# k2kobayashi/crank

Measured on AMD Instinct MI355X. Metric: train frames/sec, higher is better.
Workload: dtype bf16; 1 GPU; vqvae trainer step (all sub-updates), VCC2020-shaped synthetic 80-dim mlfb, 64 utterances x 500 frames per GPU, 14 speakers; trainer=vqvae, global_batch=64, batch_len=500, parallelism=dp1

## Files before the change

crank_amd/_lib.py:

```python
import ctypes
import os
from .config import cfg
from ctypes import c_char_p, c_double, c_float, c_int, c_longlong, c_ulonglong, c_void_p

_HERE = os.path.dirname(os.path.abspath(__file__))
LIB_PATH = cfg.lib_path or os.path.join(_HERE, "libcrank_hip.so")
_lib = None

ERRORS = {1: "invalid argument", 2: "HIP runtime error", 3: "unsupported shape/configuration"}


class NetDesc(ctypes.Structure):
    _fields_ = [
        ("kind", c_int), ("in_ch", c_int), ("out_ch", c_int), ("kernel_size", c_int), ("layers", c_int),
        ("stacks", c_int), ("res_ch", c_int), ("gate_ch", c_int), ("skip_ch", c_int), ("aux_ch", c_int),
        ("conv_ch", c_int), ("causal", c_int), ("use_bias", c_int), ("slope", c_float), ("dropout", c_float),
    ]


COLLATE_MAX_STREAMS = 8


class CollateStream(ctypes.Structure):
    _fields_ = [("src", c_void_p), ("ld", c_int), ("col0", c_int), ("ncols", c_int), ("dst", c_void_p)]


class CollateDesc(ctypes.Structure):
    _fields_ = [
        ("n_streams", c_int), ("streams", CollateStream * COLLATE_MAX_STREAMS), ("utt_start", c_void_p),
        ("utt_spk", c_void_p), ("n_utt", c_int), ("n_spk", c_int), ("lcf0_raw", c_void_p),
        ("spk_lcf0_mean", c_void_p), ("spk_lcf0_std", c_void_p), ("raw", c_void_p), ("raw_start", c_void_p),
        ("fftl", c_int), ("hop", c_int),
    ]


ADAM_MAX_BLOCKS = 4


class AdamBlock(ctypes.Structure):
    _fields_ = [("params", c_void_p), ("grads", c_void_p), ("exp_avg", c_void_p), ("exp_avg_sq", c_void_p),
                ("n", c_longlong), ("lr_dev", c_void_p), ("step_dev", c_void_p)]


class StreamDesc(ctypes.Structure):
    _fields_ = [
        ("n_stacks", c_int), ("in_ch", c_int), ("out_ch", c_int), ("emb_dim", c_int * 3), ("emb_size", c_int * 3),
        ("cb_off", c_longlong * 3), ("enc_base", c_longlong * 3), ("dec_base", c_longlong * 3), ("causal", c_int),
        ("enc_f0", c_int), ("dec_f0", c_int), ("spk_dim", c_int), ("spk_onehot", c_int), ("n_spk", c_int),
        ("spk_off", c_longlong),
    ]


class F0StreamRound(ctypes.Structure):
    _fields_ = [("ids", c_void_p), ("utt", c_void_p), ("range", c_void_p), ("chan_bf", c_void_p), ("chan", c_void_p),
                ("n_ready", c_int), ("total_samples", c_longlong), ("total_channels", c_longlong),
                ("total_frames", c_longlong), ("total_events", c_longlong)]


P, I, LL, ULL, F, D = c_void_p, c_int, c_longlong, c_ulonglong, c_float, c_double

SIGNATURES = {
    "crk_net_create": (P, [ctypes.POINTER(NetDesc)]),
    "crk_net_destroy": (None, [P]),
    "crk_net_param_count": (LL, [P]),
    "crk_net_conv_count": (I, [P]),
    "crk_net_conv_info": (I, [P, I, ctypes.POINTER(c_longlong)]),
    "crk_net_saved_bytes": (LL, [P, I, I]),
    "crk_net_reserve": (I, [P, I, I]),
    "crk_net_scratch_bytes": (LL, [P, I, I]),
    "crk_debug_alloc_count": (LL, []),
    "crk_debug_net_paths": (I, [P, I, I]),
    "crk_debug_net_partials": (LL, [P, I, I, P, LL, P]),
    "crk_seed_next": (I, [P, P, P]),
    "crk_nets_wnorm_bwd": (I, [I, P, P]),
    "crk_nets_prepare": (I, [I, P, P, ULL, P, P]),
    "crk_nets_prepare_models": (I, [I, P, P, P, I, P, P]),
    "crk_net_forward": (I, [P, P, ULL, P, I, P, I, P, I, P, I, I, I, ULL, P]),
    "crk_net_backward": (I, [P, P, ULL, P, P, I, P, I, P, I, P, I, F, P, I, P, I, I, I, ULL, P]),
    "crk_net_backward_scaled": (I, [P, P, ULL, P, P, I, P, I, P, I, P, I, F, P, I, P, I, I, I, ULL, P, P, P]),
    "crk_net_embed_grad_supported": (I, [P, I, I, I]),
    "crk_net_backward_embed": (I, [P, P, ULL, P, P, I, P, I, P, I, P, I, F, P, I, I, I, ULL, P, LL, I, I, I, P, P]),
    "crk_vq_forward": (I, [P, I, P, I, I, I, P, P, I, P, I, P]),
    "crk_vq_forward_fused": (I, [P, I, P, I, P, I, P, I, I, I, P, P, I, P, I, P, P, P, P, P]),
    "crk_vq_image_bytes": (LL, [I, I]),
    "crk_vq_image_build_multi": (I, [I, P, P, I, P, P]),
    "crk_vq_ema_scratch_bytes": (LL, [I, I, I]),
    "crk_vq_ema_stats": (I, [P, I, P, I, I, I, P, P, P, P]),
    "crk_vq_ema_apply": (I, [P, P, P, P, P, I, I, D, D, P]),
    "crk_vq_ema_partial": (I, [P, I, P, I, I, I, P, P]),
    "crk_vq_ema_reduce_multi": (I, [I, P, P, P, P, P, P, P]),
    "crk_vq_ema_apply_multi": (I, [I, P, P, P, P, P, P, P, D, D, P]),
    "crk_vq_ema_partial_multi": (I, [I, P, P, P, P, P, P, P, P]),
    "crk_vq_ema_reduce_size_multi": (I, [I, P, P, P, P, P, P, P, D, D, P]),
    "crk_vq_ema_blend_multi": (I, [I, P, P, P, P, P, P, D, P]),
    "crk_vq_ema_blend_image_multi": (I, [I, P, P, P, P, P, P, D, P, P]),
    "crk_stft_loss_multi_fwd": (I, [P, I, P, I, I, I, I, I, P, P, P, P, F, P, P, P]),
    "crk_stft_loss_multi_fwd_grad": (I, [P, I, P, I, I, I, I, I, P, P, P, P, F, P, P, I, P, P]),
    "crk_stft_loss_multi_bwd": (I, [P, I, P, I, I, I, I, I, P, P, P, P, F, P, P, I, P]),
    "crk_loss_scratch_floats": (I, []),
    "crk_masked_loss_fwd": (I, [P, I, P, I, F, P, LL, I, I, P, P, P]),
    "crk_masked_loss_bwd": (I, [P, I, P, I, F, P, LL, I, I, P, P, P, I, P, I, P]),
    "crk_masked_loss_both_fwd": (I, [P, I, P, I, P, LL, I, P, P, P]),
    "crk_weighted_sum": (I, [I, P, P, F, P, P]),
    "crk_weighted_sum_bwd": (I, [I, P, P, P, P]),
    "crk_recon_supported": (I, [I, I, P, P, P]),
    "crk_stft_twiddle_floats": (LL, [I, I]),
    "crk_stft_twiddles": (I, [I, I, P, P, P]),
    "crk_recon_grad_floats": (LL, [I, I, I, I, P, P]),
    "crk_recon_loss_fwd": (I, [P, I, P, I, P, I, I, I, I, P, P, P, P, F, P, P, P, P]),
    "crk_recon_loss_bwd": (I, [P, I, P, I, P, I, I, I, I, P, P, P, P, P, P, P, P, P, I, P]),
    "crk_masked_loss_bwd_acc": (I, [P, I, P, I, F, P, LL, I, I, P, P, P, I, P, I, P, I, P, P]),
    "crk_vq_commit_bwd": (I, [P, I, P, I, P, LL, I, P, P, P, I, P, I, P, I, P, I, P, I, P]),
    "crk_ce_fwd": (I, [P, I, P, LL, I, I, P, P, P, P]),
    "crk_ce_bwd": (I, [P, LL, I, P, P, P, P]),
    "crk_stft_loss_fwd": (I, [P, I, P, I, I, I, I, I, I, I, P, F, F, I, P, P, P]),
    "crk_stft_loss_bwd": (I, [P, I, P, I, I, I, I, I, I, I, P, F, F, P, P, I, P]),
    "crk_adam_step": (I, [P, P, P, P, LL, P, P, F, F, F, I, P]),
    "crk_adam_step_multi": (I, [I, ctypes.POINTER(AdamBlock), F, F, F, I, P]),
    "crk_radam_step": (I, [P, P, P, P, LL, P, P, D, D, D, I, P]),
    "crk_lamb_step": (I, [P, P, P, P, P, P, I, P, I, P, P, P, P, D, D, D, I, P]),
    "crk_lamb_tile": (I, []),
    "crk_concat_embed": (I, [P, I, I, P, I, I, P, I, P, LL, P, I, P]),
    "crk_embed_bwd_scratch_floats": (LL, [LL, I, I]),
    "crk_embed_bwd": (I, [P, I, I, I, P, LL, I, P, P, P]),
    "crk_concat_embed_run": (I, [P, I, I, P, I, I, P, I, P, LL, LL, P, I, P]),
    "crk_embed_bwd_run": (I, [P, I, I, I, P, LL, LL, I, P, P, P]),
    "crk_logmel_fwd": (I, [P, I, I, I, I, I, I, I, P, P, I, F, P, P, P, I, I, P]),
    "crk_logmel_stream_create": (I, [I, I, I, P, P, I, F, P, P, I, I, I, ctypes.POINTER(c_void_p)]),
    "crk_logmel_stream_destroy": (None, [P]),
    "crk_logmel_stream_state_bytes": (LL, [P]),
    "crk_logmel_stream_max_frames": (I, [P]),
    "crk_logmel_stream_reset": (I, [P, P, I, P]),
    "crk_logmel_stream_push": (I, [P, P, I, P, P, I, I, P, I, P, P]),
    "crk_scaler_apply": (I, [P, I, P, I, LL, I, P, P, I, P]),
    "crk_scaler_workspace_bytes": (LL, [I, I]),
    "crk_scaler_moments": (I, [P, I, I, I, LL, P, P, I, P, LL, P]),
    "crk_scaler_merge": (I, [P, LL, I, I, P, P, P, P, I, P, P, P, P]),
    "crk_hist_accumulate": (I, [P, LL, P, P, P, P, I, I, P, D, D, D, I, P, P, P]),
    "crk_collate_batch": (I, [ctypes.POINTER(CollateDesc), P, I, I, P, P, P, P, P, P, P, P, P]),
    "crk_decode_f0": (I, [P, P, I, I, P, P, D, D, I, P, P, P, P, P, P]),
    "crk_mcd_scratch_bytes": (LL, [I, I, I, I, I]),
    "crk_mcd_fastdtw": (I, [P, P, P, P, I, I, I, I, I, P, P, P, LL, P, P, P]),
    "crk_voc_create": (P, [I, I, I, I, P, I, P]),
    "crk_voc_destroy": (None, [P]),
    "crk_voc_workspace_bytes": (LL, [P, I, I]),
    "crk_voc_forward": (I, [P, P, P, I, I, P, P, P, LL, I, P]),
    "crk_voc_upsample": (I, [P, P, P, I, I, P, P, LL, P]),
    "crk_voc_stream_create": (I, [P, I, I, ctypes.POINTER(c_void_p)]),
    "crk_voc_stream_destroy": (None, [P]),
    "crk_voc_stream_state_bytes": (LL, [P]),
    "crk_voc_stream_lookahead": (I, [P]),
    "crk_voc_stream_reset": (I, [P, P, I, P]),
    "crk_voc_stream_push": (I, [P, P, P, P, P, I, I, P, P, I, P]),
    "crk_world_create": (P, [I, I, D, D, I, I, I]),
    "crk_world_destroy": (None, [P]),
    "crk_world_reserve": (I, [P, LL]),
    "crk_world_workspace_bytes": (LL, [P, I, LL, LL]),
# ... 122 lines not shown
```

crank_amd/csrc/loss_kernels.hip:

```cpp
#include <algorithm>
#include <type_traits>

#include "common.h"

#include "../../include/crank_hip.h"

__device__ __forceinline__ float block_sum_256(float v, float* sh) {
#pragma unroll
  for (int o = 32; o > 0; o >>= 1) v += __shfl_xor(v, o, 64);
  const int tid = threadIdx.x;
  __syncthreads();
  if ((tid & 63) == 0) sh[tid >> 6] = v;
  __syncthreads();
  return sh[0] + sh[1] + sh[2] + sh[3];
}

template <int NC>
__device__ __forceinline__ void sum_partials(const float* part, int stride, int n, float (&s)[NC], float* sh) {
#pragma unroll
  for (int j = 0; j < NC; j++) s[j] = 0.f;
  for (int i = threadIdx.x; i < n; i += 256) {
#pragma unroll
    for (int j = 0; j < NC; j++) s[j] += part[stride * i + j];
  }
// ... 952 lines not shown
            v[0] += a.x * g3; v[1 % V] += a.y * g3; v[2 % V] += a.z * g3; v[3 % V] += a.w * g3;
          } else {
            v[0] += gp[0] * g3;
          }
        }
      }
    }
    if (!p.mask || p.mask[n]) {
      float xv[V], yv[V];
      if (V == 4) {
        const float4 a = *reinterpret_cast<const float4*>(p.x + n * p.ldx + d);
        const float4 c = *reinterpret_cast<const float4*>(p.y + n * p.ldy + d);
        xv[0] = a.x; xv[1 % V] = a.y; xv[2 % V] = a.z; xv[3 % V] = a.w;
        yv[0] = c.x; yv[1 % V] = c.y; yv[2 % V] = c.z; yv[3 % V] = c.w;
      } else {
        xv[0] = p.x[n * p.ldx + d]; yv[0] = p.y[n * p.ldy + d];
      }
#pragma unroll
      for (int j = 0; j < V; j++) {
        const float df = xv[j] - yv[j];
        if (p.g1) v[j] += df > 0.f ? g1 : (df < 0.f ? -g1 : 0.f);
        if (p.g2) v[j] += 2.f * df * g2;
      }
    }
    if (V == 4) *reinterpret_cast<float4*>(p.dx + n * p.lddx + d) = make_float4(v[0], v[1 % V], v[2 % V], v[3 % V]);
    else p.dx[n * p.lddx + d] = v[0];
  }
}

extern "C" int crk_recon_loss_bwd(const float* x, int ldx, const float* y, int ldy, const unsigned char* mask, int B, int T,
                                  int D, int nres, const int* n_fft, const int* hop_length, const int* win_length,
                                  const float* out5, const float* grad, const float* g1, const float* g2, const float* g3,
                                  float* dx, int lddx, void* stream) {
  if (!x || !y || !out5 || !dx || B < 1 || T < 1 || D < 1) return CRK_ERR_ARG;
  if (g3 && (!grad || !crk_recon_supported(T, nres, n_fft, hop_length, win_length))) return CRK_ERR_ARG;
  ReconBP p;
  p.x = x; p.y = y; p.mask = mask; p.ldx = ldx; p.ldy = ldy; p.T = T; p.D = D; p.nres = g3 ? nres : 0;
  p.N = (long)B * T; p.stat = out5; p.g1 = g1; p.g2 = g2; p.g3 = g3; p.dx = dx; p.lddx = lddx;
  const float* g = grad;
  for (int r = 0; r < p.nres; r++) {
    ReconBRes& q = p.r[r];
    q.hop = hop_length[r]; q.span = win_length[r] + RC_SPAN_EXTRA; q.nf = 1 + T / q.hop;
    q.lo = n_fft[r] / 2 - (n_fft[r] - win_length[r]) / 2 + 1;
    q.gc = g;
    g += (size_t)B * q.nf * q.span * D;
  }
  const bool v4 = !((((uintptr_t)x) | ((uintptr_t)y) | ((uintptr_t)dx) | ((uintptr_t)grad)) & 15) && !((D | ldx | ldy | lddx) & 3);
  if (v4) hipLaunchKernelGGL(recon_bwd_kernel<4>, dim3(loss_blocks(p.N * (D / 4))), dim3(256), 0, (hipStream_t)stream, p);
  else hipLaunchKernelGGL(recon_bwd_kernel<1>, dim3(loss_blocks(p.N * D)), dim3(256), 0, (hipStream_t)stream, p);
  CRK_CHECK_LAUNCH();
  return CRK_OK;
}

#define WS_MAX 16
struct WsumP { const float* t[WS_MAX]; float w[WS_MAX]; int n; float c; float* out; const float* g; };
__global__ void weighted_sum_kernel(const WsumP p) {
  float s = 0.f;
#pragma unroll
  for (int i = 0; i < WS_MAX; i++)
    if (i < p.n) s += p.w[i] * p.t[i][0];
  p.out[0] = s + p.c;
}
__global__ void weighted_sum_bwd_kernel(const WsumP p) {
  const float g = p.g[0];
#pragma unroll
  for (int i = 0; i < WS_MAX; i++)
    if (i < p.n) p.out[i] = p.w[i] * g;
}
extern "C" int crk_weighted_sum(int n, const float* const* terms, const float* weights, float constant, float* out, void* stream) {
  if (n < 1 || n > WS_MAX || !terms || !weights || !out) return CRK_ERR_ARG;
  WsumP p{};
  for (int i = 0; i < n; i++) { if (!terms[i]) return CRK_ERR_ARG; p.t[i] = terms[i]; p.w[i] = weights[i]; }
  p.n = n; p.c = constant; p.out = out;
  hipLaunchKernelGGL(weighted_sum_kernel, dim3(1), dim3(1), 0, (hipStream_t)stream, p);
  CRK_CHECK_LAUNCH();
  return CRK_OK;
}
extern "C" int crk_weighted_sum_bwd(int n, const float* weights, const float* gout, float* grads, void* stream) {
  if (n < 1 || n > WS_MAX || !weights || !gout || !grads) return CRK_ERR_ARG;
  WsumP p{};
  for (int i = 0; i < n; i++) p.w[i] = weights[i];
  p.n = n; p.g = gout; p.out = grads;
  hipLaunchKernelGGL(weighted_sum_bwd_kernel, dim3(1), dim3(1), 0, (hipStream_t)stream, p);
  CRK_CHECK_LAUNCH();
  return CRK_OK;
}

template <bool CLEAR>
__global__ __launch_bounds__(256) void adam_kernel(float* __restrict__ p, float* __restrict__ g,
                                                   float* __restrict__ m, float* __restrict__ v, long n,
                                                   const float* __restrict__ lr_dev, float* __restrict__ step_dev,
                                                   float beta1, float beta2, float eps) {
  const AdamCoef c = adam_coef(lr_dev, step_dev, beta1, beta2, eps);
  for (long i = (long)blockIdx.x * 256 + threadIdx.x; i < n; i += (long)gridDim.x * 256) adam_elem<CLEAR>(p, g, m, v, i, c);
}

__global__ void adam_bump_kernel(float* step_dev) { step_dev[0] += 1.f; }

extern "C" int crk_adam_step(float* params, float* grads, float* exp_avg, float* exp_avg_sq, long long n,
                             const float* lr_dev, float* step_dev, float beta1, float beta2, float eps, int clear_grads,
                             void* stream) {
  if (!params || !grads || !exp_avg || !exp_avg_sq || !lr_dev || !step_dev) return CRK_ERR_ARG;
  hipStream_t s = (hipStream_t)stream;
  long b = (n + 255) / 256;
  if (b > 2048) b = 2048;
  if (clear_grads & 1)
    hipLaunchKernelGGL(adam_kernel<true>, dim3((int)b), dim3(256), 0, s, params, grads, exp_avg, exp_avg_sq, (long)n, lr_dev,
                       step_dev, beta1, beta2, eps);
  else
    hipLaunchKernelGGL(adam_kernel<false>, dim3((int)b), dim3(256), 0, s, params, grads, exp_avg, exp_avg_sq, (long)n, lr_dev,
                       step_dev, beta1, beta2, eps);
  if (!(clear_grads & 2)) hipLaunchKernelGGL(adam_bump_kernel, dim3(1), dim3(1), 0, s, step_dev);
  CRK_CHECK_LAUNCH();
  return CRK_OK;
}

struct AdamBlocks { crk_adam_block b[CRK_ADAM_MAX_BLOCKS]; int first[CRK_ADAM_MAX_BLOCKS + 1]; int n; };
template <bool CLEAR>
__global__ __launch_bounds__(256) void adam_multi_kernel(const AdamBlocks A, float beta1, float beta2, float eps) {
  int r = 0;
  while (r + 1 < A.n && (int)blockIdx.x >= A.first[r + 1]) r++;
  const crk_adam_block& q = A.b[r];
  const AdamCoef c = adam_coef(q.lr_dev, q.step_dev, beta1, beta2, eps);
  const long nb = A.first[r + 1] - A.first[r], n = (long)q.n;
  for (long i = (long)((int)blockIdx.x - A.first[r]) * 256 + threadIdx.x; i < n; i += nb * 256)
    adam_elem<CLEAR>(q.params, q.grads, q.exp_avg, q.exp_avg_sq, i, c);
}
struct AdamBumps { float* p[CRK_ADAM_MAX_BLOCKS]; };
__global__ void adam_bump_multi_kernel(const AdamBumps b) {
#pragma unroll
  for (int i = 0; i < CRK_ADAM_MAX_BLOCKS; i++)
    if ((int)threadIdx.x == i) b.p[i][0] += 1.f;
}
extern "C" int crk_adam_step_multi(int n_blocks, const crk_adam_block* blocks, float beta1, float beta2, float eps,
                                   int clear_grads, void* stream) {
  if (n_blocks < 1 || n_blocks > CRK_ADAM_MAX_BLOCKS || !blocks) return CRK_ERR_ARG;
  AdamBlocks A{};
// ... 266 lines not shown
```

crank_amd/net/trainer/basetrainer.py:

```python
import gc
import logging
import os
import random
from pathlib import Path

import torch

from ... import parallel
from ...config import cfg


def TrainerWrapper(trainer_type, **ka):
    from . import CycleGANTrainer, LSGANTrainer, StarGANTrainer, VQVAETrainer

    table = {"vqvae": VQVAETrainer, "lsgan": LSGANTrainer, "cyclegan": CycleGANTrainer, "stargan": StarGANTrainer}
    if trainer_type not in table:
        raise NotImplementedError("conf['trainer_type']: {} is not supported.".format(trainer_type))
    return table[trainer_type](**ka)


def to_device(batch, device):
    return {k: (v.to(device) if isinstance(v, torch.Tensor) else v) for k, v in batch.items()}


_WEIGHTS = {}


def _weight_vector(ws, like):
    key = (ws, like.device, like.dtype)
    if key not in _WEIGHTS:
        _WEIGHTS[key] = torch.tensor(ws, device=like.device, dtype=like.dtype)
    return _WEIGHTS[key]


class LossBook(dict):

    def __init__(self):
        super().__init__(objective=0.0, G=0.0, D=0.0, C=0.0, SPKRADV=0.0)
        self._pending = {}

    def add(self, key, w, term):
        self._pending.setdefault(key, []).append((float(w), term))

    def _settle(self, key):
        pend = self._pending.pop(key, None)
        if not pend:
            return
        base = super().__getitem__(key) if key in self else 0.0
        if isinstance(base, torch.Tensor):
            pend = [(1.0, base)] + pend
        tens = [(w, t) for w, t in pend if isinstance(t, torch.Tensor) and w != 0.0]
        const = sum(w * t for w, t in pend if not isinstance(t, torch.Tensor)) + (0.0 if isinstance(base, torch.Tensor) else base)
        if not tens:
            val = const
        elif len(tens) == 1 and tens[0][0] == 1.0 and const == 0.0:
            val = tens[0][1]
        elif len(tens) <= 16 and all(t.is_cuda and t.dtype == torch.float32 and t.numel() == 1 for _, t in tens):
            from ... import ops

            val = ops.weighted_sum([t for _, t in tens], [w for w, _ in tens], const)
        else:
            vec = torch.stack([t.reshape(()) for _, t in tens])
            val = (vec * _weight_vector(tuple(w for w, _ in tens), vec)).sum()
            if const != 0.0:
                val = val + const
        super().__setitem__(key, val)

    def __getitem__(self, key):
        self._settle(key)
        return super().__getitem__(key)

    def __setitem__(self, key, value):
        self._pending.pop(key, None)
        super().__setitem__(key, value)

    def items(self):
        for k in list(self._pending):
            self._settle(k)
        return super().items()

    def values(self):
        for k in list(self._pending):
            self._settle(k)
        return super().values()


class LossValues(dict):

    def __init__(self, keys, host, event, zero_keys, index=None):
        super().__init__(LossBook())
        for k in list(keys) + list(zero_keys):
            super().setdefault(k, 0.0)
        self._pending = (list(keys), host, event, index) if host is not None else None

    def _resolve(self):
        if self._pending is not None:
            keys, host, event, index = self._pending
            self._pending = None
            if event is not None:
                event.synchronize()
            vals = host.tolist()
            if index is not None:
                vals = [vals[i] for i in index]
            for k, v in zip(keys, vals):
                super().__setitem__(k, super().__getitem__(k) + v)

    def __getitem__(self, k):
        self._resolve()
        return super().__getitem__(k)

    def get(self, k, default=None):
        self._resolve()
        return super().get(k, default)

    def items(self):
        self._resolve()
        return super().items()

    def values(self):
        self._resolve()
        return super().values()

    def copy(self):
        self._resolve()
        return dict(super().items())

    def __repr__(self):
        self._resolve()
        return super().__repr__()

    def __eq__(self, other):
        self._resolve()
        return super().__eq__(other)

    __hash__ = None


def hold_collector_for_capture():
    was_on = gc.isenabled()
    for _ in range(8):
        if gc.collect() == 0:
            break
    gc.disable()
    return was_on


class GraphedStep:

    def __init__(self, trainer, batch, warmup=3, choices=()):
        refuse = cfg.test_refuse_capture_rank
        if refuse is not None and parallel.is_dist() and parallel.rank() == int(refuse):
            raise RuntimeError("capture refused on this rank (CRANK_AMD_TEST_REFUSE_CAPTURE_RANK)")
        self.trainer = trainer
        self.batch = {k: (v.clone() if isinstance(v, torch.Tensor) else v) for k, v in batch.items()}
        self.choices = tuple(choices)
        self.stream = torch.cuda.Stream()
        if warmup:
            self.stream.wait_stream(torch.cuda.current_stream())
            with torch.cuda.stream(self.stream):
                for _ in range(warmup):
                    trainer._pending_choices = list(self.choices)
                    trainer.train(self.batch)
            torch.cuda.current_stream().wait_stream(self.stream)
        torch.cuda.synchronize()
        writer, trainer.writer = trainer.writer, None
        parallel.drain_backend_watchdog()
        self.pool = torch.cuda.graph_pool_handle()
        self.segments = []
        self._ctx = None
        gc_was_on = hold_collector_for_capture()
        try:
            self._open()
            parallel._segmenter = self
            trainer._pending_choices = list(self.choices)
            try:
                self.values = trainer.train(self.batch)
            finally:
                parallel._segmenter = None
            if self.segments:
                self._tick = torch.zeros(1, device="cuda")
                self._tick.add_(1.0)
            self._close(None)
        except BaseException:
            self._abort()
            raise
        finally:
            trainer.writer = writer
            if gc_was_on:
                gc.enable()
        self._cb_state = self._codebook_state()
        self._keys = list(self.values._pending[0]) if self.values._pending else []
        self._vec = self.values._pending[1] if self.values._pending else None
        self._index = self.values._pending[3] if self.values._pending else None
        self._zero = [k for k in self.values.keys() if k not in self._keys]

    def _open(self):
        g = torch.cuda.CUDAGraph()
        mode = cfg.capture_mode
        self._ctx = (g, torch.cuda.graph(g, pool=self.pool, stream=self.stream, capture_error_mode=mode))
        self._ctx[1].__enter__()

    def _close(self, tensor):
        g, ctx = self._ctx
        self._ctx = None
        ctx.__exit__(None, None, None)
        self.segments.append((g, tensor))

    def _abort(self):
        if self._ctx is not None:
            try:
                self._ctx[1].__exit__(None, None, None)
            except Exception:
                pass
            self._ctx = None

    def collective(self, t):
        self._close(("reduce", list(t) if isinstance(t, (list, tuple)) else [t]))
        self._open()

    def collective_start(self, t):
        key = len(self.segments)
        self._close(("start", key, t))
        self._open()
        return key

    def collective_finish(self, key):
        self._close(("finish", key))
        self._open()

    def _codebook_state(self):
        return tuple(getattr(m, "codebook_epoch", -1) for m in self.trainer.model.values())

    def step(self, batch=None):
        if self._codebook_state() != self._cb_state:
            for m in self.trainer.model.values():
                if hasattr(m, "refresh_images"):
                    m.refresh_images(force=True)
            self._cb_state = self._codebook_state()
        if batch is not None:
            for k, v in batch.items():
                if isinstance(v, torch.Tensor):
                    self.batch[k].copy_(v, non_blocking=True)
                else:
                    self.batch[k] = v
        inflight = {}
        for g, act in self.segments:
            g.replay()
            if act is None:
                continue
            if act[0] == "reduce":
                for t in act[1]:
                    parallel.all_reduce_now(t)
            elif act[0] == "start":
                inflight[act[1]] = parallel.all_reduce_async(act[2])
            else:
                work = inflight.pop(act[1], None)
                if work is not None:
                    work.wait()
        if self._vec is None:
            return LossValues(self._keys, None, None, self._zero)
        host = torch.empty(self._vec.shape, dtype=self._vec.dtype, pin_memory=True)
        host.copy_(self._vec, non_blocking=True)
        done = torch.cuda.Event()
        done.record()
        return LossValues(self._keys, host, done, self._zero, self._index)


class BaseTrainer(object):
    def __init__(self, model, optimizer, criterion, dataloader, writer, expdir, conf, feat_conf, scheduler=None,
                 scaler=None, resume=0, device="cuda", n_jobs=-1):
        self.model, self.optimizer, self.criterion = model, optimizer, criterion
        self._graphs = {}
        self._pending_choices = None
        if parallel.is_dist():
            self.criterion = parallel.wrap_criterion(criterion)
        self.dataloader, self.writer = dataloader, writer
        self.expdir = Path(expdir)
        self.conf, self.feat_conf = conf, feat_conf
        self.scheduler, self.scaler = scheduler, scaler
        self.device, self.n_jobs = device, n_jobs
        self.spkrs = dataloader["spkrs"]
        self.n_spkrs = len(self.spkrs)
        self.resume_steps = self.steps = resume
        self._step_schedulers(explicit=True)
        self.finish_train = False
        self.rng = random.Random()
        self.rng.setstate(random.getstate())

    def run(self, flag="train", tdir=None):
        self.flag = flag
        if flag != "train":
            return self._run_eval(flag)
        while not self.finish_train:
            self._tr_step()
        logging.info("Finish training")

    def _mode_signature(self):
        return tuple(sorted((k, v) for k, v in vars(self).items()
                            if (k.endswith("_flag") or k == "stop_generator") and isinstance(v, bool)))

    def _draw_step_choices(self):
        return ()

    def _choose(self, options):
        if self._pending_choices:
            return self._pending_choices.pop(0)
        return self.rng.choice(options)

    def train_graphed(self, batch):
        choices = tuple(self._draw_step_choices())
        if self._graphs is None:
            self._pending_choices = list(choices)
            return self.train(batch)
# ... 44 lines not shown
                break

    def _dev_step(self):
        ds = self.conf["dev_steps"]
        if self.steps % ds == 0 and self.steps > ds - 1 and self.steps != self.resume_steps and "dev" in self.dataloader:
            values = None
            for i, batch in enumerate(self.dataloader["dev"]):
                values = self.dev(to_device(batch, self.device))
                if i > 0:
                    break
            if values is not None:
                self._print_loss_values(values, phase="dev")

    def _run_eval(self, flag):
        out = []
        if flag == "eval":
            for batch in self.dataloader["eval"]:
                out.append(self.eval(to_device(batch, self.device)))
        elif flag == "reconstruction":
            for key in ["train", "dev"]:
                for batch in self.dataloader[key]:
                    out.append(self.reconstruction(to_device(batch, self.device)))
        return out

    def _step_schedulers(self, explicit=False):
        if self.scheduler is None:
            return
        scheds = self.scheduler.values() if isinstance(self.scheduler, dict) else [self.scheduler]
        for s in scheds:
            s.step(self.steps)

    def save_model(self):
        self.expdir.mkdir(parents=True, exist_ok=True)
        state = {"steps": self.steps, "model": {"G": self.model["G"].state_dict()}}
        for m in ["SPKRADV", "D", "C"]:
            if m in self.model:
                state["model"][m] = self.model[m].state_dict()
        torch.save(state, self.expdir / "checkpoint_{}steps.pkl".format(self.steps))

    def check_custom_start(self):
        pass

    def _get_loss_dict(self, batch=None):
        if batch is not None:
            parallel.prepare_step(batch, self.conf)
        return LossBook()

    def _parse_loss(self, loss):
        keys = [k for k, v in loss.items() if isinstance(v, torch.Tensor)]
        others = [k for k in loss if k not in keys]
        if not keys:
            return LossValues(keys, None, None, others)
        index = None if parallel.is_dist() else self._arena_index([loss[k] for k in keys])
        if index is not None:
            vec = self._arena.buf
        else:
            vec = torch.stack([loss[k].detach().reshape(()).float() for k in keys])
        if parallel.is_dist():
            parallel.all_reduce_sum(vec)
        if not vec.is_cuda:
            return LossValues(keys, vec, None, others)
        if torch.cuda.is_current_stream_capturing():
            return LossValues(keys, vec, None, others, index)
        host = torch.empty(vec.shape, dtype=vec.dtype, pin_memory=True)
        host.copy_(vec, non_blocking=True)
        done = torch.cuda.Event()
        done.record()
        return LossValues(keys, host, done, others, index)

    _arena = None

    def _open_arena(self):
        from ... import ops

        self._arena = ops.begin_scalar_arena(self.device if torch.device(self.device).type == "cuda" else None)

    def _close_arena(self):
        from ... import ops

        ops.begin_scalar_arena(None)
        self._cond_cache = self._label_cache = None

    def _arena_index(self, tensors):
        a = self._arena
        if a is None:
            return None
        base = a.buf.untyped_storage().data_ptr()
        index = []
        for t in tensors:
            if not (t.is_cuda and t.dtype == torch.float32 and t.numel() == 1 and t.untyped_storage().data_ptr() == base):
                return None
            index.append(t.storage_offset() - a.buf.storage_offset())
        return index

    def _print_loss_values(self, values, phase="train"):
        logging.info("{} iterations: {}".format(phase, self.steps))
        for k, v in sorted(values.items()):
            if v != 0.0:
                logging.info("{}: {}".format(k, v))

    def _flush_writer(self, loss, phase):
        if self.writer is None or self.steps % self.conf["n_steps_print_loss"] != 0:
            return
        w = self.writer.get(phase) if isinstance(self.writer, dict) else None
        if w is None:
            return
        for k, v in loss.items():
            if isinstance(v, torch.Tensor):
                w.add_scalar("loss/{}".format(k), v.item(), self.steps)
        w.flush()

    def _get_enc_h(self, batch, use_cvfeats=False, cv_spkr_name=None):
        if self.conf["encoder_f0"]:
            return self._get_f0_condition(batch, cv_spkr_name, use_cvfeats)
        return None

    def _get_dec_h(self, batch, use_cvfeats=False, cv_spkr_name=None):
        h, h_onehot = self._get_spkr_conditions(batch, cv_spkr_name, use_cvfeats)
        if not self.conf["use_spkr_embedding"]:
            f0 = self._get_f0_condition(batch, cv_spkr_name, use_cvfeats) if self.conf["decoder_f0"] else None
            return (torch.cat([f0, h_onehot], dim=-1) if f0 is not None else h_onehot), None
        pair = getattr(self.model.get("G"), "can_pair_f0", False)
        f0 = self._get_f0_condition(batch, cv_spkr_name, use_cvfeats, pair=pair) if self.conf["decoder_f0"] else None
        return f0, h

    def _get_f0_condition(self, batch, cv_spkr_name, use_cvfeats=False, pair=False):
        if cv_spkr_name is not None:
            lcf0 = self._get_cvf0(batch, cv_spkr_name)
# ... 129 lines not shown
```

crank_amd/ops.py:

```python
import ctypes

import torch

from . import _lib
from .config import cfg
from ._lib import check, ptr, stream_ptr

_PRECISION = cfg.precision


def set_precision(name):
    global _PRECISION
    if name not in ("bf16", "bf16x3", "bf16x3f"):
        raise ValueError(f"unknown precision {name!r} (bf16 | bf16x3 | bf16x3f)")
    _PRECISION = name


def get_precision():
    return _PRECISION


CRK_FLAG_PRECISE = 1
CRK_FLAG_NO_PARAM_GRAD = 2
CRK_FLAG_NO_SAVE = 4
CRK_FLAG_DEFER_WNORM = 8
CRK_FLAG_SEED_ON_DEVICE = 16
CRK_FLAG_FWD_PRECISE = 32
CRK_FLAG_BWD_PLAIN = 64


def _flags(skip_param_grads=False, no_save=False, precision=None, defer_wnorm=False, backward=False):
    prec = precision or _PRECISION
    if prec == "bf16x3f":
        pbits = CRK_FLAG_FWD_PRECISE if backward else (CRK_FLAG_PRECISE | CRK_FLAG_BWD_PLAIN)
    else:
        pbits = CRK_FLAG_PRECISE if prec == "bf16x3" else 0
    return (pbits | (CRK_FLAG_NO_PARAM_GRAD if skip_param_grads else 0) | (CRK_FLAG_NO_SAVE if no_save else 0)
            | (CRK_FLAG_DEFER_WNORM if defer_wnorm else 0))


class _ScalarArena:

    def __init__(self, device, n=256):
        self.buf = torch.empty(n, device=device, dtype=torch.float32)
        self.pos = 0


_ARENA = None


def begin_scalar_arena(device):
    global _ARENA
    dev = torch.device(device) if device is not None else None
    _ARENA = _ScalarArena(dev) if (dev is not None and dev.type == "cuda") else None
    return _ARENA


def scalar_arena():
    return _ARENA


def _scalars(n, device):
    a = _ARENA
    if a is not None and a.buf.device == device and a.pos + n <= a.buf.numel():
        t = a.buf[a.pos: a.pos + n]
        a.pos += (n + 3) & ~3
        return t
    return torch.empty(n, device=device, dtype=torch.float32)


def _rows(t):
    assert t.dtype == torch.float32, t.dtype
    if t.dim() == 3:
        B, T, C = t.shape
        if t.stride(2) == 1 and (B == 1 or t.stride(0) == T * t.stride(1)) and t.stride(1) >= C:
            return t, t.stride(1)
    elif t.dim() == 2:
        if t.stride(1) == 1 and t.stride(0) >= t.size(1):
            return t, t.stride(0)
    t = t.contiguous()
    return t, t.size(-1)


class HipNet:

    def __init__(self, **desc):
        L = _lib.lib()
        self.desc = _lib.NetDesc(**desc)
        self.handle = L.crk_net_create(ctypes.byref(self.desc))
        if not self.handle:
            raise RuntimeError(f"crk_net_create failed for {desc}")
        self.n_params = L.crk_net_param_count(self.handle)
        self.convs = []
        buf = (ctypes.c_longlong * 9)()
        for i in range(L.crk_net_conv_count(self.handle)):
            check(L.crk_net_conv_info(self.handle, i, buf), "crk_net_conv_info")
            self.convs.append(tuple(int(v) for v in buf))
        self.in_ch, self.out_ch = desc["in_ch"], desc["out_ch"]
        self.aux_ch = desc.get("aux_ch", 0)
        self.dropout = float(desc.get("dropout", 0.0))
        self._saved_bytes = {}
        self.seed_state = None
        if self.dropout > 0:
            self.reseed(int(torch.randint(0, 2 ** 62, (1,)).item()))

    def reseed(self, value):
        from . import parallel
# ... 747 lines not shown
        ctx.save_for_backward(xk, yk, mk if mk is not None else out, out)
        return out[0], out[2], out[4]

    @staticmethod
    def backward(ctx, g1, g2, g3):
        L = _lib.lib()
        xk, yk, mk, out = ctx.saved_tensors
        N, Dm, ldx, ldy = ctx.geom
        mk = mk if ctx.has_m else None
        unit, ctx.unit = ctx.unit, None
        if g3 is not None and unit is None:
            raise RuntimeError("the STFT term of a recon loss can be differentiated once")
        if g1 is None and g2 is None and g3 is None:
            return None, None, None, None, None, None
        if ctx.fused:
            B, T = xk.shape[0], xk.shape[1]
            ia = _res_arrays(ctx.res)
            gs = [None if g is None else g.contiguous().reshape(1) for g in (g1, g2, g3)]
            dx = torch.empty(N, Dm, device=xk.device, dtype=torch.float32)
            check(L.crk_recon_loss_bwd(ptr(xk), ldx, ptr(yk), ldy, ptr(mk), B, T, Dm, len(ctx.res), ia[0], ia[1], ia[2],
                                       ptr(out), ptr(unit), ptr(gs[0]), ptr(gs[1]), ptr(gs[2]), ptr(dx), Dm, stream_ptr()),
                  "crk_recon_loss_bwd")
            return dx.view(ctx.xshape), None, None, None, None, None
        dx, scale = (unit, g3.contiguous().reshape(1)) if g3 is not None else (None, None)
        dx, scale = _masked_bwd_acc(xk, yk, mk, ctx.geom, out, (g1, g2), dx, scale)
        if scale is not None:
            dx = dx.mul_(scale)
        return dx.view(ctx.xshape), None, None, None, None, None


def recon_loss(x, y, mask, resolutions, windows, logratio=0.0):
    return _ReconFn.apply(x, y, mask, tuple(resolutions), tuple(windows), logratio)


def stft_loss(x, y, resolutions, windows, logratio=0.0):
    return _STFTLossFn.apply(x, y, tuple(resolutions), tuple(windows), logratio)


_ONES = {}
_WCONST = {}


def one_like(t):
    key = (t.device, t.dtype, tuple(t.shape))
    if key not in _ONES:
        _ONES[key] = torch.ones_like(t)
    return _ONES[key]


def _farr(vals):
    return (ctypes.c_float * len(vals))(*[float(v) for v in vals])


class _WeightedSumFn(torch.autograd.Function):

    @staticmethod
    def forward(ctx, weights, constant, *terms):
        ts = [t.reshape(1) if t.is_contiguous() else t.contiguous().reshape(1) for t in terms]
        out = _scalars(1, terms[0].device)
        check(_lib.lib().crk_weighted_sum(len(ts), _parr(ts), _farr(weights), float(constant), ptr(out), stream_ptr()),
              "crk_weighted_sum")
        ctx.weights = tuple(float(w) for w in weights)
        return out[0]

    @staticmethod
    def backward(ctx, g):
        ws = ctx.weights
        one = _ONES.get((g.device, g.dtype, tuple(g.shape)))
        key = (ws, g.device)
        cached = one is not None and g.data_ptr() == one.data_ptr()
        if cached and key not in _WCONST:
            if g.is_cuda and torch.cuda.is_current_stream_capturing():
                cached = False
            else:
                _WCONST[key] = torch.tensor(ws, device=g.device, dtype=torch.float32)
        if cached:
            grads = _WCONST[key]
        else:
            grads = torch.empty(len(ws), device=g.device, dtype=torch.float32)
            check(_lib.lib().crk_weighted_sum_bwd(len(ws), _farr(ws), ptr(g.contiguous().reshape(1)), ptr(grads), stream_ptr()),
                  "crk_weighted_sum_bwd")
        return (None, None) + tuple(grads[i] for i in range(len(ws)))


def weighted_sum(terms, weights, constant=0.0):
    return _WeightedSumFn.apply(tuple(weights), float(constant), *terms)


def _label_runs(idx):
    B, T = idx.shape
    if T > 1 and idx.stride(1) == 0 and (B == 1 or idx.stride(0) == T):
        return idx, T
    return idx.contiguous(), 1


def _concat_embed_fwd(a, b, table, idx):
    L = _lib.lib()
    B, T = idx.shape
    ak, lda = (None, 0) if a is None else _rows(a)
    bk, ldb = (None, 0) if b is None else _rows(b)
    ca = 0 if a is None else a.shape[-1]
    cb = 0 if b is None else b.shape[-1]
    E = table.shape[1]
    out = torch.empty(B, T, ca + cb + E, device=idx.device, dtype=torch.float32)
    ik, run = _label_runs(idx)
    check(L.crk_concat_embed_run(ptr(ak), lda, ca, ptr(bk), ldb, cb, ptr(table), E, ptr(ik), run, B * T, ptr(out),
                                 ca + cb + E, stream_ptr()), "crk_concat_embed_run")
    return out, ik, run, (ca, cb, E)


class _ConcatEmbedFn(torch.autograd.Function):

    @staticmethod
    def forward(ctx, a, b, table, idx, owner, tab_offset, flat):
# ... 98 lines not shown
```

include/crank_hip.h:

```cpp
#ifndef CRANK_HIP_H
#define CRANK_HIP_H
#ifdef __cplusplus
extern "C" {
#endif

#define CRK_OK 0
#define CRK_ERR_ARG 1
#define CRK_ERR_HIP 2
#define CRK_ERR_UNSUPPORTED 3

#define CRK_FLAG_PRECISE 1
#define CRK_FLAG_NO_PARAM_GRAD 2
#define CRK_FLAG_NO_SAVE 4
#define CRK_FLAG_DEFER_WNORM 8

#define CRK_FLAG_SEED_ON_DEVICE 16
#define CRK_FLAG_FWD_PRECISE 32
#define CRK_FLAG_BWD_PLAIN 64

typedef struct crk_net_desc {
  int kind;
  int in_ch, out_ch, kernel_size, layers, stacks;
  int res_ch, gate_ch, skip_ch, aux_ch;
  int conv_ch;
// ... 66 lines not shown
                                 void* stream);

int crk_loss_scratch_floats(void);
int crk_masked_loss_fwd(const float* x, int ldx, const float* y, int ldy, float yconst, const unsigned char* mask,
                        long long N, int D, int mode, float* out2, float* scratch, void* stream);
int crk_masked_loss_bwd(const float* x, int ldx, const float* y, int ldy, float yconst, const unsigned char* mask,
                        long long N, int D, int mode, const float* stat2, const float* gout, float* dx, int lddx,
                        float* dy, int lddy, void* stream);
int crk_masked_loss_both_fwd(const float* x, int ldx, const float* y, int ldy, const unsigned char* mask, long long N,
                             int D, float* out4, float* scratch, void* stream);
int crk_masked_loss_bwd_acc(const float* x, int ldx, const float* y, int ldy, float yconst, const unsigned char* mask,
                            long long N, int D, int mode, const float* stat2, const float* gout, float* dx, int lddx,
                            float* dy, int lddy, const float* add, int ldadd, const float* add_scale, void* stream);
int crk_vq_commit_bwd(const float* x, int ldx, const float* e, int lde, const unsigned char* mask, long long N, int D,
                      const float* stat2, const float* gout, float* dx, int lddx, float* dsum, int ldsum,
                      const float* a1, int ld1, const float* a2, int ld2, const float* a3, int ld3, void* stream);
int crk_ce_fwd(const float* logits, int ldl, const long long* target, long long N, int C, int ignore_index,
               float* out2, float* dlogits_unscaled, float* scratch, void* stream);
int crk_ce_bwd(float* dlogits_unscaled, long long N, int C, const float* stat2, const float* gout, float* dlogits,
               void* stream);
int crk_stft_loss_fwd(const float* x, int ldx, const float* y, int ldy, int B, int T, int D, int n_fft,
                      int hop_length, int win_length, const float* window, float logratio, float weight,
                      int accumulate, float* out1, float* scratch, void* stream);
int crk_stft_loss_bwd(const float* x, int ldx, const float* y, int ldy, int B, int T, int D, int n_fft,
                      int hop_length, int win_length, const float* window, float logratio, float weight,
                      const float* gout, float* dx, int lddx, void* stream);

int crk_stft_loss_multi_fwd(const float* x, int ldx, const float* y, int ldy, int B, int T, int D, int nres,
                            const int* n_fft, const int* hop_length, const int* win_length, const float* const* windows,
                            float logratio, float* out1, float* scratch, void* stream);
int crk_stft_loss_multi_fwd_grad(const float* x, int ldx, const float* y, int ldy, int B, int T, int D, int nres,
                                 const int* n_fft, const int* hop_length, const int* win_length,
                                 const float* const* windows, float logratio, float* out1, float* dx_unit, int lddx,
                                 float* scratch, void* stream);
int crk_stft_loss_multi_bwd(const float* x, int ldx, const float* y, int ldy, int B, int T, int D, int nres,
                            const int* n_fft, const int* hop_length, const int* win_length, const float* const* windows,
                            float logratio, const float* gout, float* dx, int lddx, void* stream);

int crk_recon_supported(int T, int nres, const int* n_fft, const int* hop_length, const int* win_length);
long long crk_stft_twiddle_floats(int n_fft, int win_length);
int crk_stft_twiddles(int n_fft, int win_length, const float* window, float* table, void* stream);
long long crk_recon_grad_floats(int B, int T, int D, int nres, const int* hop_length, const int* win_length);
int crk_recon_loss_fwd(const float* x, int ldx, const float* y, int ldy, const unsigned char* mask, int B, int T, int D,
                       int nres, const int* n_fft, const int* hop_length, const int* win_length,
                       const float* const* tables, float logratio, float* out5, float* grad, float* scratch,
                       void* stream);
int crk_recon_loss_bwd(const float* x, int ldx, const float* y, int ldy, const unsigned char* mask, int B, int T, int D,
                       int nres, const int* n_fft, const int* hop_length, const int* win_length, const float* out5,
                       const float* grad, const float* g1, const float* g2, const float* g3, float* dx, int lddx,
                       void* stream);

int crk_weighted_sum(int n, const float* const* terms, const float* weights, float constant, float* out, void* stream);
int crk_weighted_sum_bwd(int n, const float* weights, const float* gout, float* grads, void* stream);

int crk_adam_step(float* params, float* grads, float* exp_avg, float* exp_avg_sq, long long n, const float* lr_dev,
                  float* step_dev, float beta1, float beta2, float eps, int clear_grads, void* stream);
#define CRK_ADAM_MAX_BLOCKS 4
typedef struct crk_adam_block {
  float *params, *grads, *exp_avg, *exp_avg_sq;
  long long n;
  const float* lr_dev;
  float* step_dev;
} crk_adam_block;
int crk_adam_step_multi(int n_blocks, const crk_adam_block* blocks, float beta1, float beta2, float eps, int clear_grads,
                        void* stream);
int crk_radam_step(float* params, float* grads, float* exp_avg, float* exp_avg_sq, long long n, const float* lr_dev,
                   float* step_dev, double beta1, double beta2, double eps, int clear_grads, void* stream);
int crk_lamb_step(float* params, float* grads, float* exp_avg, float* exp_avg_sq, float* upd, const int* tiles, int n_tiles,
                  const int* tensors, int n_tensors, float* part, float* ratio_out, const float* lr_dev, float* step_dev,
                  double beta1, double beta2, double eps, int clear_grads, void* stream);
int crk_lamb_tile(void);
int crk_concat_embed(const float* a, int lda, int ca, const float* b, int ldb, int cb, const float* table, int E,
                     const long long* idx, long long N, float* out, int ldo, void* stream);
long long crk_embed_bwd_scratch_floats(long long N, int E, int n_rows);
int crk_embed_bwd(const float* dcat, int ld, int c0, int E, const long long* idx, long long N, int n_rows,
                  float* dtable, float* scratch, void* stream);
int crk_concat_embed_run(const float* a, int lda, int ca, const float* b, int ldb, int cb, const float* table, int E,
                         const long long* idx, long long run, long long N, float* out, int ldo, void* stream);
int crk_embed_bwd_run(const float* dcat, int ld, int c0, int E, const long long* idx, long long run, long long N,
                      int n_rows, float* dtable, float* scratch, void* stream);

int crk_logmel_fwd(const float* raw, int ld_raw, int B, int n_samples, int T, int n_fft, int hop, int win_length,
                   const float* window, const float* mel_basis , int n_mels, float eps,
                   const float* mean, const float* std, float* out, int ldo, int center, void* stream);

int crk_logmel_stream_create(int n_fft, int hop, int win_length, const float* window, const float* mel_basis, int n_mels,
                             float eps, const float* mean, const float* stdv, int center, int n_streams, int max_samples,
                             void** handle);
void crk_logmel_stream_destroy(void* st);
long long crk_logmel_stream_state_bytes(void* st);
int crk_logmel_stream_max_frames(void* st);
int crk_logmel_stream_reset(void* st, const int* stream_ids, int n, void* stream);
int crk_logmel_stream_push(void* st, const float* x, int ldx, const int* n_valid, const int* end, int S, int C, float* out,
                           int ldo, int* n_frames, void* stream);


int crk_scaler_apply(const float* x, int ldx, float* y, int ldy, long long N, int D, const double* mean,
                     const double* scale, int inverse, void* stream);

long long crk_scaler_workspace_bytes(int U, int D);
int crk_scaler_moments(const float* x, int ld, int col0, int D, long long F_total, const long long* utt_start,
                       const long long* utt_start_host, int U, void* workspace, long long workspace_bytes,
                       void* stream);
int crk_scaler_merge(const void* workspace, long long workspace_bytes, int U, int D, const long long* group_start,
                     const int* group_utts, const long long* group_start_host, const int* group_utts_host, int G,
                     double* mean, double* var, long long* count, void* stream);
// ... 223 lines not shown
```

Measured before the change: 22.17 million frames/s.

## Publish loss scalars to a pinned host ring from the captured graph

When the train step is captured as a single graph, weighted loss sums are deferred into one final kernel. That kernel computes them, then writes the scalar arena straight into a pinned host ring buffer and bumps a replay counter. This replaces the per-step pinned-host copy and event, and the several tiny weighted-sum launches, with one launch. Host readers spin on the published counter, falling back to a stream sync after a timeout. It adds host-side spin-waiting, ring-slot retirement logic and a zero-copy system-memory write.

```diff
diff --git a/crank_amd/_lib.py b/crank_amd/_lib.py
--- a/crank_amd/_lib.py
+++ b/crank_amd/_lib.py
@@ -40,6 +40,15 @@
 class AdamBlock(ctypes.Structure):
     _fields_ = [("params", c_void_p), ("grads", c_void_p), ("exp_avg", c_void_p), ("exp_avg_sq", c_void_p),
                 ("n", c_longlong), ("lr_dev", c_void_p), ("step_dev", c_void_p)]
+
+
+WSUM_MAX = 16
+PUBLISH_MAX_DEFERRED = 8
+
+
+class Wsum(ctypes.Structure):
+    _fields_ = [("t", c_void_p * WSUM_MAX), ("w", c_float * WSUM_MAX), ("n", c_int), ("c", c_float), ("out", c_void_p),
+                ("g", c_void_p)]
 
 
 class StreamDesc(ctypes.Structure):
@@ -103,6 +112,8 @@
     "crk_masked_loss_both_fwd": (I, [P, I, P, I, P, LL, I, P, P, P]),
     "crk_weighted_sum": (I, [I, P, P, F, P, P]),
     "crk_weighted_sum_bwd": (I, [I, P, P, P, P]),
+    "crk_publish_scalars": (I, [P, I, P, I, P, P, ctypes.POINTER(Wsum), I, P]),
+    "crk_host_device_pointer": (I, [P, ctypes.POINTER(c_void_p)]),
     "crk_recon_supported": (I, [I, I, P, P, P]),
     "crk_stft_twiddle_floats": (LL, [I, I]),
     "crk_stft_twiddles": (I, [I, I, P, P, P]),
diff --git a/crank_amd/csrc/loss_kernels.hip b/crank_amd/csrc/loss_kernels.hip
--- a/crank_amd/csrc/loss_kernels.hip
+++ b/crank_amd/csrc/loss_kernels.hip
@@ -1028,15 +1028,16 @@
   return CRK_OK;
 }
 
-#define WS_MAX 16
-struct WsumP { const float* t[WS_MAX]; float w[WS_MAX]; int n; float c; float* out; const float* g; };
-__global__ void weighted_sum_kernel(const WsumP p) {
+#define WS_MAX CRK_WSUM_MAX
+typedef crk_wsum WsumP;
+__device__ __forceinline__ void weighted_sum_body(const WsumP& p) {
   float s = 0.f;
 #pragma unroll
   for (int i = 0; i < WS_MAX; i++)
     if (i < p.n) s += p.w[i] * p.t[i][0];
   p.out[0] = s + p.c;
 }
+__global__ void weighted_sum_kernel(const WsumP p) { weighted_sum_body(p); }
 __global__ void weighted_sum_bwd_kernel(const WsumP p) {
   const float g = p.g[0];
 #pragma unroll
@@ -1059,6 +1060,55 @@
   p.n = n; p.g = gout; p.out = grads;
   hipLaunchKernelGGL(weighted_sum_bwd_kernel, dim3(1), dim3(1), 0, (hipStream_t)stream, p);
   CRK_CHECK_LAUNCH();
+  return CRK_OK;
+}
+
+#define PUB_THREADS 64
+struct PublishP {
+  const float* arena; int n; float* ring; int slots; unsigned long long *count, *host_count; int nd;
+  WsumP d[CRK_PUBLISH_MAX_DEFERRED];
+};
+__global__ __launch_bounds__(PUB_THREADS) void publish_scalars_kernel(const PublishP p) {
+  if (threadIdx.x == 0)
+    for (int k = 0; k < p.nd; k++) weighted_sum_body(p.d[k]);
+  __syncthreads();
+  const unsigned long long count = p.count[0];
+  float* slot = p.ring + (size_t)(count % (unsigned long long)p.slots) * p.n;
+  for (int i = threadIdx.x; i < p.n; i += PUB_THREADS) slot[i] = p.arena[i];
+  __threadfence_system();
+  __syncthreads();
+  if (threadIdx.x == 0) {
+    p.count[0] = count + 1;
+    if (p.host_count) p.host_count[0] = count + 1;
+  }
+}
+extern "C" int crk_publish_scalars(const float* arena, int n, float* host_ring, int slots, unsigned long long* replay_count,
+                                   unsigned long long* host_count, const crk_wsum* deferred, int n_deferred, void* stream) {
+  if (!arena || n < 1 || !host_ring || slots < 1 || !replay_count) return CRK_ERR_ARG;
+  if (n_deferred < 0 || n_deferred > CRK_PUBLISH_MAX_DEFERRED || (n_deferred && !deferred)) return CRK_ERR_ARG;
+  PublishP p{};
+  p.arena = arena; p.n = n; p.ring = host_ring; p.slots = slots; p.count = replay_count; p.host_count = host_count;
+  p.nd = n_deferred;
+  for (int k = 0; k < n_deferred; k++) {
+    const WsumP& d = deferred[k];
+    if (d.n < 1 || d.n > WS_MAX || !d.out) return CRK_ERR_ARG;
+    for (int i = 0; i < d.n; i++)
+      if (!d.t[i]) return CRK_ERR_ARG;
+    p.d[k] = d;
+  }
+  hipLaunchKernelGGL(publish_scalars_kernel, dim3(1), dim3(PUB_THREADS), 0, (hipStream_t)stream, p);
+  CRK_CHECK_LAUNCH();
+  return CRK_OK;
+}
+extern "C" int crk_host_device_pointer(const void* host, void** dev) {
+  if (!host || !dev) return CRK_ERR_ARG;
+  hipPointerAttribute_t a;
+  if (hipPointerGetAttributes(&a, host) != hipSuccess) {
+    (void)hipGetLastError();
+    return CRK_ERR_UNSUPPORTED;
+  }
+  if (a.type != hipMemoryTypeHost || !a.devicePointer) return CRK_ERR_UNSUPPORTED;
+  dev[0] = a.devicePointer;
   return CRK_OK;
 }
 
diff --git a/crank_amd/net/trainer/basetrainer.py b/crank_amd/net/trainer/basetrainer.py
--- a/crank_amd/net/trainer/basetrainer.py
+++ b/crank_amd/net/trainer/basetrainer.py
@@ -2,6 +2,8 @@
 import logging
 import os
 import random
+import time
+import weakref
 from pathlib import Path
 
 import torch
@@ -105,6 +107,13 @@
             for k, v in zip(keys, vals):
                 super().__setitem__(k, super().__getitem__(k) + v)
 
+    def _retire(self):
+        if self._pending is not None:
+            keys, host, event, index = self._pending
+            if event is not None:
+                event.synchronize()
+            self._pending = (keys, host.clone(), None, index)
+
     def __getitem__(self, k):
         self._resolve()
         return super().__getitem__(k)
@@ -134,6 +143,53 @@
         return super().__eq__(other)
 
     __hash__ = None
+
+
+class PublishRing:
+
+    def __init__(self, rows, published):
+        self.rows = rows
+        self.slots = rows.shape[0]
+        self.published = published
+        self.patience = 1.0
+        self.replays = 0
+        self._live = [None] * self.slots
+
+    def claim(self):
+        slot = self.replays % self.slots
+        ref, self._live[slot] = self._live[slot], None
+        old = ref() if ref is not None else None
+        if old is not None:
+            old._retire()
+        return slot
+
+    def values(self, slot, keys, stream, zero_keys, index):
+        vals = LossValues(keys, self.rows[slot], _Landed(self, self.replays, stream), zero_keys, index)
+        vals.replay = self.replays
+        self._live[slot] = weakref.ref(vals)
+        self.replays += 1
+        return vals
+
+    def wait(self, replay, stream):
+        need = replay + 2
+        if need <= self.replays:
+            deadline = time.monotonic() + self.patience
+            while time.monotonic() < deadline:
+                if int(self.published[0]) >= need:
+                    return
+        stream.synchronize()
+
+
+class _Landed:
+
+    def __init__(self, ring, replay, stream):
+        self.ring, self.replay, self.stream = ring, replay, stream
+
+    def synchronize(self):
+        self.ring.wait(self.replay, self.stream)
+
+
+PUBLISH_SLOTS = 8
 
 
 def hold_collector_for_capture():
@@ -165,6 +221,15 @@
         torch.cuda.synchronize()
         writer, trainer.writer = trainer.writer, None
         parallel.drain_backend_watchdog()
+        self._ring = None
+        publish = not parallel.is_dist() and torch.device(trainer.device).type == "cuda"
+        if publish:
+            from ... import ops
+            store = torch.zeros(PUBLISH_SLOTS, 256, dtype=torch.float32, pin_memory=True)
+            ring_ptr = ops.host_device_pointer(store)
+            self._count = torch.zeros(1, dtype=torch.int64, device=trainer.device)
+            self._published = torch.zeros(1, dtype=torch.int64, pin_memory=True)
+            published_ptr = ops.host_device_pointer(self._published)
         self.pool = torch.cuda.graph_pool_handle()
         self.segments = []
         self._ctx = None
@@ -173,10 +238,21 @@
             self._open()
             parallel._segmenter = self
             trainer._pending_choices = list(self.choices)
+            trainer._publish_follows = publish
             try:
                 self.values = trainer.train(self.batch)
             finally:
                 parallel._segmenter = None
+                trainer._publish_follows = False
+            pend = self.values._pending
+            arena = trainer._arena if publish else None
+            if arena is not None and not self.segments and pend is not None and pend[3] is not None and pend[1] is arena.buf:
+                n = arena.pos
+                ops.publish_scalars(arena.buf, n, ring_ptr, PUBLISH_SLOTS, self._count, arena.deferred, published_ptr)
+                arena.deferred = []
+                self._ring = PublishRing(store.view(-1)[: PUBLISH_SLOTS * n].view(PUBLISH_SLOTS, n), self._published)
+            elif arena is not None and arena.deferred:
+                raise RuntimeError("loss totals were left to a publish launch that does not follow")
             if self.segments:
                 self._tick = torch.zeros(1, device="cuda")
                 self._tick.add_(1.0)
@@ -243,6 +319,7 @@
                     self.batch[k].copy_(v, non_blocking=True)
                 else:
                     self.batch[k] = v
+        slot = self._ring.claim() if self._ring is not None else None
         inflight = {}
         for g, act in self.segments:
             g.replay()
@@ -259,6 +336,8 @@
                     work.wait()
         if self._vec is None:
             return LossValues(self._keys, None, None, self._zero)
+        if slot is not None:
+            return self._ring.values(slot, self._keys, torch.cuda.current_stream(), self._zero, self._index)
         host = torch.empty(self._vec.shape, dtype=self._vec.dtype, pin_memory=True)
         host.copy_(self._vec, non_blocking=True)
         done = torch.cuda.Event()
@@ -409,6 +488,9 @@
         if not keys:
             return LossValues(keys, None, None, others)
         index = None if parallel.is_dist() else self._arena_index([loss[k] for k in keys])
+        if index is None and self._arena is not None and self._arena.deferred:
+            from ... import ops
+            ops.flush_deferred_sums()
         if index is not None:
             vec = self._arena.buf
         else:
@@ -426,11 +508,13 @@
         return LossValues(keys, host, done, others, index)
 
     _arena = None
+    _publish_follows = False
 
     def _open_arena(self):
         from ... import ops
 
-        self._arena = ops.begin_scalar_arena(self.device if torch.device(self.device).type == "cuda" else None)
+        self._arena = ops.begin_scalar_arena(self.device if torch.device(self.device).type == "cuda" else None,
+                                             defer_sums=self._publish_follows)
 
     def _close_arena(self):
         from ... import ops
diff --git a/crank_amd/ops.py b/crank_amd/ops.py
--- a/crank_amd/ops.py
+++ b/crank_amd/ops.py
@@ -41,18 +41,23 @@
 
 class _ScalarArena:
 
-    def __init__(self, device, n=256):
+    def __init__(self, device, n=256, defer_sums=False):
         self.buf = torch.empty(n, device=device, dtype=torch.float32)
         self.pos = 0
+        self.defer_sums = defer_sums
+        self.deferred = []
+
+    def owns(self, t):
+        return t.untyped_storage().data_ptr() == self.buf.untyped_storage().data_ptr()
 
 
 _ARENA = None
 
 
-def begin_scalar_arena(device):
+def begin_scalar_arena(device, defer_sums=False):
     global _ARENA
     dev = torch.device(device) if device is not None else None
-    _ARENA = _ScalarArena(dev) if (dev is not None and dev.type == "cuda") else None
+    _ARENA = _ScalarArena(dev, defer_sums=defer_sums) if (dev is not None and dev.type == "cuda") else None
     return _ARENA
 
 
@@ -906,14 +911,51 @@
     return (ctypes.c_float * len(vals))(*[float(v) for v in vals])
 
 
+def _launch_weighted_sum(ts, weights, constant, out):
+    check(_lib.lib().crk_weighted_sum(len(ts), _parr(ts), _farr(weights), float(constant), ptr(out), stream_ptr()),
+          "crk_weighted_sum")
+
+
+def flush_deferred_sums():
+    a = _ARENA
+    if a is None or not a.deferred:
+        return
+    pending, a.deferred = a.deferred, []
+    for ts, weights, constant, out in pending:
+        _launch_weighted_sum(ts, weights, constant, out)
+
+
+def host_device_pointer(t):
+    dev = ctypes.c_void_p()
+    check(_lib.lib().crk_host_device_pointer(t.data_ptr(), ctypes.byref(dev)), "crk_host_device_pointer")
+    return dev.value
+
+
+def publish_scalars(arena, n, ring_ptr, slots, count, deferred=(), published_ptr=0):
+    assert arena.dtype == torch.float32 and arena.is_contiguous() and 1 <= n <= arena.numel()
+    assert count.dtype == torch.int64 and count.numel() == 1 and count.device == arena.device
+    recs = (_lib.Wsum * max(len(deferred), 1))()
+    for r, (ts, weights, constant, out) in zip(recs, deferred):
+        for i, (t, w) in enumerate(zip(ts, weights)):
+            r.t[i], r.w[i] = t.data_ptr(), w
+        r.n, r.c, r.out = len(ts), constant, out.data_ptr()
+    check(_lib.lib().crk_publish_scalars(ptr(arena), int(n), ring_ptr, int(slots), ptr(count), published_ptr, recs,
+                                         len(deferred), stream_ptr()), "crk_publish_scalars")
+
+
 class _WeightedSumFn(torch.autograd.Function):
 
     @staticmethod
     def forward(ctx, weights, constant, *terms):
         ts = [t.reshape(1) if t.is_contiguous() else t.contiguous().reshape(1) for t in terms]
         out = _scalars(1, terms[0].device)
-        check(_lib.lib().crk_weighted_sum(len(ts), _parr(ts), _farr(weights), float(constant), ptr(out), stream_ptr()),
-              "crk_weighted_sum")
+        a = _ARENA
+        if (a is not None and a.defer_sums and a.owns(out) and len(a.deferred) < _lib.PUBLISH_MAX_DEFERRED
+                and torch.cuda.is_current_stream_capturing()):
+            a.deferred.append((ts, tuple(float(w) for w in weights), float(constant), out))
+        else:
+            flush_deferred_sums()
+            _launch_weighted_sum(ts, weights, constant, out)
         ctx.weights = tuple(float(w) for w in weights)
         return out[0]
 
diff --git a/include/crank_hip.h b/include/crank_hip.h
--- a/include/crank_hip.h
+++ b/include/crank_hip.h
@@ -142,6 +142,19 @@
 
 int crk_weighted_sum(int n, const float* const* terms, const float* weights, float constant, float* out, void* stream);
 int crk_weighted_sum_bwd(int n, const float* weights, const float* gout, float* grads, void* stream);
+#define CRK_WSUM_MAX 16
+typedef struct crk_wsum {
+  const float* t[CRK_WSUM_MAX];
+  float w[CRK_WSUM_MAX];
+  int n;
+  float c;
+  float* out;
+  const float* g;
+} crk_wsum;
+#define CRK_PUBLISH_MAX_DEFERRED 8
+int crk_publish_scalars(const float* arena, int n, float* host_ring, int slots, unsigned long long* replay_count,
+                        unsigned long long* host_count, const crk_wsum* deferred, int n_deferred, void* stream);
+int crk_host_device_pointer(const void* host, void** dev);
 
 int crk_adam_step(float* params, float* grads, float* exp_avg, float* exp_avg_sq, long long n, const float* lr_dev,
                   float* step_dev, float beta1, float beta2, float eps, int clear_grads, void* stream);
```

Measured after the change: 22.32 million frames/s, median of 6. Within noise of the previous version (+0.7%).
